# kensho-technologies/pyctcdecode

Measured on AMD Instinct MI355X. Metric: logit-frames/sec (whole node) at beam=100, V=1024, 4-gram LM, higher is better.
Workload: dtype f64

## Files before the change

### pyctcdecode_amd/csrc/backend_hip.hip

```cpp
#include <hip/hip_runtime.h>
#include <hip/hip_fp16.h>
#include <algorithm>
#include <type_traits>
#include <vector>
#include <math.h>
#include <stdio.h>
#include <stdlib.h>

#include "backend.h"
#include "beam_core.h"
#include "beam_wave.h"
#include "set_order.h"
#include "np_f32.h"
#include "set_order_small.h"
#include "np_sum.h"
#include "text_wave.h"
#include "wave_ops_hip.h"

namespace ctc {
namespace be {

static hipStream_t g_stream = nullptr;
static hipStream_t g_copy_stream = nullptr;
static hipEvent_t g_ev[3] = {nullptr, nullptr, nullptr};
// ... 1147 lines not shown
        Raw v;
        v.x = xf[e0 < V ? e0 : 0];
        v.y = xf[e0 + 1 < V ? e0 + 1 : 0];
        v.z = xf[e0 + 2 < V ? e0 + 2 : 0];
        v.w = xf[e0 + 3 < V ? e0 + 3 : 0];
        r[k] = v;
      } else {
        r[k] = x4[i4 < n4 ? i4 : 0];
      }
    }
  };
  auto widen = [&](const Raw(&raw)[NL], float4(&r)[NC]) {
    const float ninf = -INFINITY;
    if constexpr (WIDE) {
#pragma unroll
      for (int k = 0; k < NC; ++k) {
        r[k] = make_float4(raw[k].x, raw[k].y, raw[k].z, raw[k].w);
        if constexpr (!AL) {
          const int e0 = (k * 64 + lane) * 4;
          if (e0 >= V) r[k].x = ninf;
          if (e0 + 1 >= V) r[k].y = ninf;
          if (e0 + 2 >= V) r[k].z = ninf;
          if (e0 + 3 >= V) r[k].w = ninf;
        } else if (!in_row(k)) {
          r[k] = make_float4(ninf, ninf, ninf, ninf);
        }
      }
    } else {
#pragma unroll
      for (int k = 0; k < NL; ++k) {
        r[2 * k] = make_float4(pf_widen<DT>(raw[k].x & 0xFFFFu), pf_widen<DT>(raw[k].x >> 16), pf_widen<DT>(raw[k].y & 0xFFFFu),
                               pf_widen<DT>(raw[k].y >> 16));
        r[2 * k + 1] = make_float4(pf_widen<DT>(raw[k].z & 0xFFFFu), pf_widen<DT>(raw[k].z >> 16), pf_widen<DT>(raw[k].w & 0xFFFFu),
                                   pf_widen<DT>(raw[k].w >> 16));
        if (!in_row(2 * k)) {
          r[2 * k] = make_float4(ninf, ninf, ninf, ninf);
          r[2 * k + 1] = make_float4(ninf, ninf, ninf, ninf);
        }
      }
    }
  };

  float my_m = 0.f, my_rs = 0.f, my_s32 = 1.0f;
  double my_s = 1.0;
  int my_first = 0;
  uint32_t my_cnt = 0;

  int np_off0 = 0, np_len0 = 0;
  if constexpr (NP) {
    const int leaf = lane >> 3;
    if (leaf < a.np_n_leaf) {
      np_off0 = a.np_leaf[2 * leaf];
      np_len0 = a.np_leaf[2 * leaf + 1];
    }
  }
  auto np_accumulate = [&](int i) {
#ifdef CTC_NP_DIAG_NOEXCH
    if (lane < a.np_n_leaf) np_ls[lane * PF_ROWS + i] = 1.0f;
    return;
#endif
    __builtin_amdgcn_fence(__ATOMIC_SEQ_CST, "wavefront");
    __builtin_amdgcn_wave_barrier();
    const int g = lane >> 3, j = lane & 7;
    const int nl = a.np_n_leaf;
    for (int base = 0; base < nl; base += 8) {
      const int leaf = base + g;
      const bool mine = leaf < nl;
      int off = np_off0, len = np_len0;
      if (base > 0) {
        off = len = 0;
        if (mine) {
          off = a.np_leaf[2 * leaf];
          len = a.np_leaf[2 * leaf + 1];
        }
      }
      float res = 0.f;
      if (len == 128 && (off & 127) == 0) {
        const float* q = np_rb + np_pad(off) + j;
        float t0 = q[0], t1 = q[8], t2 = q[16], t3 = q[24], t4 = q[32], t5 = q[40], t6 = q[48], t7 = q[56];
        float t8 = q[64], t9 = q[72], t10 = q[80], t11 = q[88], t12 = q[96], t13 = q[104], t14 = q[112], t15 = q[120];
        float rr = t0 + t1;
        rr = rr + t2; rr = rr + t3; rr = rr + t4; rr = rr + t5; rr = rr + t6; rr = rr + t7; rr = rr + t8;
        rr = rr + t9; rr = rr + t10; rr = rr + t11; rr = rr + t12; rr = rr + t13; rr = rr + t14; rr = rr + t15;
        res = rr;
      } else if (len >= 8) {
        const int body = len - (len & 7);
        float rr = np_rb[np_pad(off + j)];
        for (int t = 8; t < body; t += 8) rr = rr + np_rb[np_pad(off + t + j)];
        res = rr;
      }
      res = res + dpp_f32<0xB1, 0xf>(0.f, res);
      res = res + dpp_f32<0x4E, 0xf>(0.f, res);
      res = res + dpp_f32<0x141, 0xf>(0.f, res);
      if ((len & 7) != 0 || len < 8) {
        const int body = len >= 8 ? len - (len & 7) : 0;
        if (len < 8) res = 0.f;
        for (int t = body; t < len; ++t) res = res + np_rb[np_pad(off + t)];
      }
      if (a.np_uniform8) {
        float t = res + dpp_f32<0x128, 0xf>(0.f, res);
        t = t + dpp_f32<0x142, 0xa>(0.f, t);
        t = t + dpp_f32<0x143, 0xc>(0.f, t);
        const float total = __int_as_float(__builtin_amdgcn_readlane(__float_as_int(t), 63));
        if (lane == i) my_s32 = total;
      } else if (mine && j == 0) {
        np_ls[leaf * PF_ROWS + i] = res;
      }
    }
    __builtin_amdgcn_fence(__ATOMIC_SEQ_CST, "wavefront");
    __builtin_amdgcn_wave_barrier();
  };

  auto phase_a = [&](int i, const Raw(&raw)[NL]) -> uint32_t {
    float4 r[NC];
    widen(raw, r);
    float mf = -INFINITY, rsf;
#pragma unroll
    for (int k = 0; k < NC; ++k) mf = max3_raw(max3_raw(mf, r[k].x, r[k].y), r[k].z, r[k].w);
    if (!AL) {
      rsf = 0.f;
#pragma unroll
      for (int k = 0; k < NC; ++k) {
        const int e0 = (k * 64 + lane) * 4;
        rsf += ((e0 < V ? r[k].x : 0.f) + (e0 + 1 < V ? r[k].y : 0.f)) + ((e0 + 2 < V ? r[k].z : 0.f) + (e0 + 3 < V ? r[k].w : 0.f));
      }
    } else if (n4 == NL * 64) {
      f32x2 rs2 = (f32x2)(0.f);
#pragma unroll
      for (int k = 0; k < NC; ++k) rs2 += (f32x2){r[k].x, r[k].y} + (f32x2){r[k].z, r[k].w};
      rsf = rs2.x + rs2.y;
    } else {
      rsf = 0.f;
#pragma unroll
      for (int k = 0; k < NC; ++k) rsf += in_row(k) ? (r[k].x + r[k].y) + (r[k].z + r[k].w) : 0.f;
    }
    const float m = wave_max_f32(mf);
    const float rs = wave_sum_f32(rsf);
    uint32_t cnt = 0xFFFFu;
    int first = 0;
    double s = 1.0;
    bool clean = isfinite(m) && rs == rs;
    if constexpr (NP) {
      float lo = INFINITY;
#pragma unroll
      for (int k = 0; k < NC; ++k) {
        if constexpr (AL) {
          if (n4 == NL * 64 || in_row(k)) lo = min3_raw(min3_raw(lo, r[k].x, r[k].y), r[k].z, r[k].w);
        } else {
          const int e0 = (k * 64 + lane) * 4;
          lo = fminf(lo, fminf(fminf(e0 < V ? r[k].x : lo, e0 + 1 < V ? r[k].y : lo), fminf(e0 + 2 < V ? r[k].z : lo, e0 + 3 < V ? r[k].w : lo)));
        }
      }
      if (clean && __ballot(!(lo - m > -87.0f)) != 0ull) clean = false;
    }
    if (clean) {
      if constexpr (NP) {
        f32x2 approx = (f32x2)(0.f);
        const f32x2 mm2 = (f32x2)(m);
#if !defined(CTC_NP_DIAG_PKEXP) && !defined(CTC_NP_CHAINWISE)
#ifndef CTC_NP_IL
#define CTC_NP_IL 2
#endif
        constexpr int IL = NC % CTC_NP_IL == 0 ? CTC_NP_IL : 1;
        f32x2 ex[NC][2];
#pragma unroll
        for (int k0 = 0; k0 < NC; k0 += IL) {
          f32x2 tin[2 * IL], tout[2 * IL];
#pragma unroll
          for (int j = 0; j < IL; ++j) {
            tin[2 * j] = (f32x2){r[k0 + j].x, r[k0 + j].y} - mm2;
            tin[2 * j + 1] = (f32x2){r[k0 + j].z, r[k0 + j].w} - mm2;
          }
          np_exp_nonpos_pk_fast_n<2 * IL>(tin, tout);
#pragma unroll
          for (int j = 0; j < IL; ++j) {
            ex[k0 + j][0] = tout[2 * j];
            ex[k0 + j][1] = tout[2 * j + 1];
          }
        }
#endif
#pragma unroll
        for (int k = 0; k < NC; ++k) {
#ifdef CTC_NP_DIAG_PKEXP
          const f32x2 e01 = exp_nonpos_f32x2m((f32x2){r[k].x, r[k].y} - mm2), e23 = exp_nonpos_f32x2m((f32x2){r[k].z, r[k].w} - mm2);
#elif defined(CTC_NP_CHAINWISE)
          const f32x2 e01 = np_exp_nonpos_pk_fast((f32x2){r[k].x, r[k].y} - mm2), e23 = np_exp_nonpos_pk_fast((f32x2){r[k].z, r[k].w} - mm2);
#else
          const f32x2 e01 = ex[k][0], e23 = ex[k][1];
#endif
          bool inside = true;
          if constexpr (AL) inside = n4 == NL * 64 || in_row(k);
          else inside = (k * 64 + lane) * 4 + 3 < V;
          if (inside) approx += e01 + e23;
#ifndef CTC_NP_DIAG_NOEXCH
          *(float4*)(np_rb + np_pad((k * 64 + lane) * 4)) = make_float4(e01.x, e01.y, e23.x, e23.y);
#endif
        }
        s = (double)wave_sum_f32(approx.x + approx.y);
      } else {
      f32x2 acc = (f32x2)(0.f);
      const f32x2 mm = (f32x2)(m);
#pragma unroll
      for (int k = 0; k < NC; ++k) {
#ifdef CTC_PF_SKIP_EXP
        acc += ((f32x2){r[k].x, r[k].y} - mm) * (f32x2)(1e-9f) + ((f32x2){r[k].z, r[k].w} - mm) * (f32x2)(1e-9f);
#else
        acc += exp_nonpos_f32x2m((f32x2){r[k].x, r[k].y} - mm);
        acc += exp_nonpos_f32x2m((f32x2){r[k].z, r[k].w} - mm);
#endif
      }
      s = wave_sum((double)(acc.x + acc.y));
#ifdef CTC_PF_SKIP_EXP
      s = 1.02 + s * 1e-30;
#endif
      }
      const float xthr = (m + __logf((float)s)) + tminf;
      const float pre = xthr - 3e-5f * (4.0f + fabsf(xthr));
      cnt = 0;
#pragma unroll
      for (int k = 0; k < NC; ++k) {
#pragma unroll
        for (int e = 0; e < 4; ++e) {
          const float x = e == 0 ? r[k].x : e == 1 ? r[k].y : e == 2 ? r[k].z : r[k].w;
          const bool c = x >= pre;
          const uint64_t mk = __ballot(c);
          if (mk) {
            const uint32_t pos = cnt + lanes_below(mk);
            if (c && pos < (uint32_t)PF_CAND) {
              ar_id[pos * PF_ROWS + i] = (uint16_t)id_of(k, e);
              ar_x[pos * PF_ROWS + i] = x;
            }
            cnt += (uint32_t)__popcll(mk);
          }
        }
      }
      if (cnt == 0) {
        first = 0x7FFFFFFF;
#pragma unroll
        for (int k = 0; k < NC; ++k) {
          if (first == 0x7FFFFFFF || (!WIDE && (k & 1))) {
            const uint64_t b0 = __ballot(r[k].x == m), b1 = __ballot(r[k].y == m), b2 = __ballot(r[k].z == m),
                           b3 = __ballot(r[k].w == m);
            const uint64_t any = b0 | b1 | b2 | b3;
            if (any) {
              const int l = __builtin_ctzll(any);
              const int e = ((b0 >> l) & 1ull) ? 0 : ((b1 >> l) & 1ull) ? 1 : ((b2 >> l) & 1ull) ? 2 : 3;
              const int cand = WIDE ? (k * 64 + l) * 4 + e : ((k >> 1) * 64 + l) * 8 + (k & 1) * 4 + e;
              if (cand < first) first = cand;
            }
          }
        }
      }
      if constexpr (NP) np_accumulate(i);
    }
    if (lane == i) {
      my_m = m;
      my_rs = rs;
      my_s = s;
      my_first = first;
      my_cnt = cnt;
    }
    return cnt;
  };

  const int64_t row_last = row_lo + nrows - 1;
  auto row_at = [&](int i) { return row_lo + i < row_last ? row_lo + i : row_last; };
  if constexpr (NC <= 4) {
    Raw ra[NL], rb[NL], rc[NL];
    load_row(row_at(0), ra);
    load_row(row_at(1), rb);
    for (int i = 0; i < nrows; i += 3) {
      load_row(row_at(i + 2), rc);
      phase_a(i, ra);
      load_row(row_at(i + 3), ra);
      if (i + 1 < nrows) phase_a(i + 1, rb);
      load_row(row_at(i + 4), rb);
      if (i + 2 < nrows) phase_a(i + 2, rc);
    }
  } else if constexpr (NC <= 8) {
    Raw ra[NL], rb[NL];
    load_row(row_at(0), ra);
    for (int i = 0; i < nrows; i += 2) {
      load_row(row_at(i + 1), rb);
      phase_a(i, ra);
      load_row(row_at(i + 2), ra);
      if (i + 1 < nrows) phase_a(i + 1, rb);
    }
  } else {
    Raw ra[NL];
    for (int i = 0; i < nrows; ++i) {
      load_row(row_at(i), ra);
      phase_a(i, ra);
    }
  }
  __syncthreads();

  const int64_t row = row_lo + lane;
  const uint32_t ms = (uint32_t)a.max_surv;
  bool slow = false;
#ifdef CTC_PF_SKIP_B
  if (lane < nrows) {
    a.surv_id[(size_t)row * ms] = 0;
    a.surv_lp[(size_t)row * ms] = -1.0 + 1e-30 * (double)(my_cnt + (uint32_t)my_first) + 1e-30 * my_s;
    a.surv_cnt[row] = 1;
    a.row_sum[row] = (double)my_rs + (double)my_m * 1e-30;
  }
#else
  if (lane < nrows) {
    const uint32_t cnt = my_cnt;
    slow = cnt > (uint32_t)PF_CAND;
    if (!slow) {
      const double s = my_s;
      const double md = (double)my_m;
      double lse = 0.0;
      float l32 = 0.f;
      if constexpr (NP) {
        float s32 = my_s32;
        if (!a.np_uniform8) {
          for (int q = 0; q + 1 < a.np_n_leaf; ++q) {
            const int dst = a.np_prog[2 * q], src = a.np_prog[2 * q + 1];
            np_ls[dst * PF_ROWS + lane] = np_ls[dst * PF_ROWS + lane] + np_ls[src * PF_ROWS + lane];
          }
          s32 = np_ls[lane];
        }
        l32 = np_log_f32(s32);
      } else {
        lse = log_ge1(s);
      }
      auto logp_of = [&](float x) { return NP ? to_logp_np32(x, false, my_m, l32) : to_logp((double)x, false, md, lse); };
      const double best = logp_of(my_m);
      uint16_t* ids = ar_id + lane;
      float* xs = ar_x + lane;
      uint32_t n = 0;
      uint32_t first = cnt > 0 ? 0xFFFFu : (uint32_t)my_first;
      for (uint32_t j = 0; j < cnt; ++j) {
        const uint16_t id = ids[j * PF_ROWS];
        const float x = xs[j * PF_ROWS];
        if (x == my_m && id < first) first = id;
        if (logp_of(x) >= a.token_min_logp) {
          uint32_t p = n;
          while (p > 0 && ids[(p - 1) * PF_ROWS] > id) {
            ids[p * PF_ROWS] = ids[(p - 1) * PF_ROWS];
            xs[p * PF_ROWS] = xs[(p - 1) * PF_ROWS];
            --p;
          }
          ids[p * PF_ROWS] = id;
          xs[p * PF_ROWS] = x;
          ++n;
        }
      }
      slow = n > SMALL_SET_MAX_KEYS || n >= ms;
      if (!slow) {
        LaneTab tab{tabs + lane};
        const SmallSet r = small_set_order(tab, n, [ids](uint32_t k) { return (uint32_t)ids[k * PF_ROWS]; },
                                           first);
        uint16_t* out_id = a.surv_id + (size_t)row * ms;
        double* out_lp = a.surv_lp + (size_t)row * ms;
        uint32_t pos = 0;
        for (uint32_t k = 0; k <= r.mask; ++k) {
          const uint16_t v = tab.get(r.base + k);
          if (v != SMALL_SET_EMPTY) {
            const uint32_t pay = v >> SMALL_SET_ID_BITS;
            out_id[pos] = (uint16_t)(v & SMALL_SET_ID_MASK);
            out_lp[pos] = pay == SMALL_SET_ARGMAX ? best : logp_of(xs[pay * PF_ROWS]);
            ++pos;
          }
        }
        a.surv_cnt[row] = pos;
        a.row_sum[row] = (double)my_rs;
      }
    }
  }
#endif
  const uint64_t sm = __ballot(slow);
  if (sm) {
    uint32_t base = 0;
    if (lane == 0) base = atomicAdd(&a.overflow[3], (uint32_t)__popcll(sm));
    base = (uint32_t)__builtin_amdgcn_readfirstlane((int)base);
    if (slow) a.slow_rows[base + lanes_below(sm)] = (uint32_t)(row - a.row_base);
  }
}

struct NpPlan {
  int V = -1, n_leaf = 0, uniform8 = 0;
  uint16_t* d_leaf = nullptr;
  uint8_t* d_prog = nullptr;
};
static int np_plan_node(int off, int n, std::vector<uint16_t>& leaf, std::vector<uint8_t>& prog) {
  if (n <= 128) {
    leaf.push_back((uint16_t)off);
    leaf.push_back((uint16_t)n);
    return (int)leaf.size() / 2 - 1;
  }
  int n2 = n / 2;
  n2 -= n2 % 8;
  const int l = np_plan_node(off, n2, leaf, prog), r = np_plan_node(off + n2, n - n2, leaf, prog);
  prog.push_back((uint8_t)l);
  prog.push_back((uint8_t)r);
  return l;
}
static int np_plan_for(int V, NpPlan** out, std::string* err) {
  static NpPlan plans[4];
  static int next = 0;
  for (NpPlan& p : plans)
    if (p.V == V) {
      *out = &p;
      return 0;
    }
  NpPlan& p = plans[next];
  next = (next + 1) % 4;
  std::vector<uint16_t> leaf;
  std::vector<uint8_t> prog;
  np_plan_node(0, V, leaf, prog);
  prog.push_back(0);
  prog.push_back(0);
  HIP_TRY(hipStreamSynchronize(g_stream));
  if (p.d_leaf) (void)hipFree(p.d_leaf);
  if (p.d_prog) (void)hipFree(p.d_prog);
  p.d_leaf = nullptr;
  p.d_prog = nullptr;
  p.V = -1;
  HIP_TRY(hipMalloc((void**)&p.d_leaf, leaf.size() * 2));
  HIP_TRY(hipMalloc((void**)&p.d_prog, prog.size()));
  HIP_TRY(hipMemcpy(p.d_leaf, leaf.data(), leaf.size() * 2, hipMemcpyHostToDevice));
  HIP_TRY(hipMemcpy(p.d_prog, prog.data(), prog.size(), hipMemcpyHostToDevice));
  p.n_leaf = (int)leaf.size() / 2;
  p.uniform8 = (p.n_leaf == 1 || p.n_leaf == 2 || p.n_leaf == 4 || p.n_leaf == 8) ? 1 : 0;
  for (size_t k = 0; k < leaf.size(); k += 2)
    if (leaf[k + 1] != 128 || (leaf[k] & 127) != 0) p.uniform8 = 0;
  p.V = V;
  *out = &p;
  return 0;
}

int launch_prune(const PruneArgs& a_in, std::string* err) {
  PruneArgs a = a_in;
  {
    const char* ex0 = getenv("CTCDEC_PRUNE_EXP");
    a.f32_np = (a.dtype == 0 && !(ex0 && (ex0[0] == 'p' || ex0[0] == 'f'))) ? 1 : 0;
    a.np_prog = nullptr;
    a.np_leaf = nullptr;
    a.np_n_leaf = 0;
    a.np_uniform8 = 0;
  }
  if (a.pass == 0) {
    g_timing_valid = false;
    HIP_TRY(hipEventRecord(g_ev[0], g_stream));
  }
  if (a.n_rows > 0) {
    uint32_t cap = set_table_cap((uint32_t)a.max_surv + 1);
    size_t lds = prune_lds_bytes((size_t)a.max_surv, cap) * PRUNE_WAVES;
    if (lds > 160 * 1024) {
      if (err) *err = "token_min_logp admits too many labels per frame for the LDS set tables";
      return -1;
    }
    dim3 grid((unsigned)((a.n_rows + PRUNE_WAVES - 1) / PRUNE_WAVES)), block(PRUNE_WAVES * 64);
    const bool vec4 = a.dtype == 0 && (a.n_labels % 4) == 0 && a.n_labels <= 1024 && a.rows_aligned16;
    static_assert(PF_MAX_LABELS - 1 <= (int)SMALL_SET_MAX_ID, "label ids must fit the small set tables");
    const bool f32_fast = a.dtype == 0 && a.n_labels <= PF_MAX_LABELS && a.rows_aligned4;
    const bool f32_al = (a.n_labels % 4) == 0 && a.rows_aligned16;
#define CTC_LAUNCH_PRUNE(KERN)                                                                                 \
  do {                                                                                                         \
    HIP_TRY(hipFuncSetAttribute((const void*)KERN, hipFuncAttributeMaxDynamicSharedMemorySize, (int)lds));      \
    hipLaunchKernelGGL(KERN, grid, block, lds, g_stream, a, cap);                                              \
  } while (0)
    const char* ex = getenv("CTCDEC_PRUNE_EXP");
    const char* pk = getenv("CTCDEC_PRUNE_KERNEL");
    const bool rows_ok = a.pass == 0 && a.slow_rows && a.n_rows < (1ll << 32) && !(ex && ex[0] == 'f') && !(pk && pk[0] == 'r') &&
                         !(a.dense_hint && a.dtype == 0 && a.f32_np);
    const bool rows64 = f32_fast && rows_ok;
    const bool rows64h = (a.dtype == 2 || a.dtype == 3) && (a.n_labels % 8) == 0 && a.n_labels <= 1024 && a.rows_aligned16 && rows_ok;
    const dim3 fgrid((unsigned)((a.n_rows + PF_ROWS - 1) / PF_ROWS)), fblock(64);
    const unsigned rest = (unsigned)std::min<int64_t>((a.n_rows + PRUNE_WAVES - 1) / PRUNE_WAVES, 2048);
    if (rows64) {
      const int nc = ((a.n_labels + 3) / 4 + 63) / 64;
      size_t flds = PF_LDS;
      if (a.f32_np) {
        NpPlan* plan = nullptr;
        if (np_plan_for(a.n_labels, &plan, err)) return -1;
        a.np_leaf = plan->d_leaf;
        a.np_prog = plan->d_prog;
        a.np_n_leaf = plan->n_leaf;
        a.np_uniform8 = plan->uniform8;
        flds += pf_np_extra_lds(nc <= 8 ? nc : (nc <= 12 ? 12 : 16), plan->uniform8 ? 0 : plan->n_leaf);
      }
#define CTC_LAUNCH_FAST_K(KERN)                                                                                           \
  do {                                                                                                                    \
    HIP_TRY(hipFuncSetAttribute((const void*)KERN, hipFuncAttributeMaxDynamicSharedMemorySize, (int)flds));               \
    hipLaunchKernelGGL(KERN, fgrid, fblock, flds, g_stream, a);                                                           \
  } while (0)
#define CTC_LAUNCH_FAST(NCV, ALV)                                                                                         \
  do {                                                                                                                    \
    if (a.f32_np) CTC_LAUNCH_FAST_K((frame_prune_fast<NCV, 0, ALV, true>));                                               \
    else CTC_LAUNCH_FAST_K((frame_prune_fast<NCV, 0, ALV, false>));                                                       \
    if (ALV && NCV <= 4) {                                                                                                \
      HIP_TRY(hipFuncSetAttribute((const void*)frame_prune_f32x4_listed<(NCV <= 4 ? NCV : 4)>,                            \
                                  hipFuncAttributeMaxDynamicSharedMemorySize, (int)lds));                                 \
      hipLaunchKernelGGL((frame_prune_f32x4_listed<(NCV <= 4 ? NCV : 4)>), dim3(rest), block, lds, g_stream, a, cap);     \
    } else {                                                                                                              \
      HIP_TRY(hipFuncSetAttribute((const void*)frame_prune_listed<float>, hipFuncAttributeMaxDynamicSharedMemorySize,     \
                                  (int)lds));                                                                             \
      hipLaunchKernelGGL((frame_prune_listed<float>), dim3(rest), block, lds, g_stream, a, cap);                          \
    }                                                                                                                     \
  } while (0)
#define CTC_LAUNCH_FAST_NC(NCV)            \
  do {                                     \
    if (f32_al) CTC_LAUNCH_FAST(NCV, true); \
    else CTC_LAUNCH_FAST(NCV, false);      \
  } while (0)
      switch (nc) {
        case 1: CTC_LAUNCH_FAST_NC(1); break;
        case 2: CTC_LAUNCH_FAST_NC(2); break;
        case 3: CTC_LAUNCH_FAST_NC(3); break;
        case 4: CTC_LAUNCH_FAST_NC(4); break;
        case 5: CTC_LAUNCH_FAST_NC(5); break;
        case 6: CTC_LAUNCH_FAST_NC(6); break;
        case 7: CTC_LAUNCH_FAST_NC(7); break;
        case 8: CTC_LAUNCH_FAST_NC(8); break;
        case 9: case 10: case 11: case 12: CTC_LAUNCH_FAST_NC(12); break;
        default: CTC_LAUNCH_FAST_NC(16); break;
      }
#undef CTC_LAUNCH_FAST_NC
#undef CTC_LAUNCH_FAST
#undef CTC_LAUNCH_FAST_K
    } else if (rows64h) {
      const int nl = (a.n_labels / 8 + 63) / 64;
#define CTC_LAUNCH_FAST16(NCV, DTV, T)                                                                                    \
  do {                                                                                                                    \
    hipLaunchKernelGGL((frame_prune_fast<NCV, DTV>), fgrid, fblock, PF_LDS, g_stream, a);                                 \
    HIP_TRY(hipFuncSetAttribute((const void*)frame_prune_listed<T>, hipFuncAttributeMaxDynamicSharedMemorySize, (int)lds)); \
    hipLaunchKernelGGL((frame_prune_listed<T>), dim3(rest), block, lds, g_stream, a, cap);                                 \
  } while (0)
      if (a.dtype == 2) {
        if (nl <= 1) CTC_LAUNCH_FAST16(2, 2, half_bits);
        else CTC_LAUNCH_FAST16(4, 2, half_bits);
      } else {
        if (nl <= 1) CTC_LAUNCH_FAST16(2, 3, bf16_bits);
        else CTC_LAUNCH_FAST16(4, 3, bf16_bits);
      }
#undef CTC_LAUNCH_FAST16
    } else if (vec4) {
      const int nc = (a.n_labels / 4 + 63) / 64;
      if (!(ex && ex[0] == 'f')) {
        if (nc <= 1) CTC_LAUNCH_PRUNE((frame_prune_f32x4<1, true>));
        else if (nc == 2) CTC_LAUNCH_PRUNE((frame_prune_f32x4<2, true>));
        else if (nc == 3) CTC_LAUNCH_PRUNE((frame_prune_f32x4<3, true>));
        else CTC_LAUNCH_PRUNE((frame_prune_f32x4<4, true>));
      } else {
        if (nc <= 1) CTC_LAUNCH_PRUNE((frame_prune_f32x4<1, false>));
        else if (nc == 2) CTC_LAUNCH_PRUNE((frame_prune_f32x4<2, false>));
        else if (nc == 3) CTC_LAUNCH_PRUNE((frame_prune_f32x4<3, false>));
        else CTC_LAUNCH_PRUNE((frame_prune_f32x4<4, false>));
      }
    } else if (a.dtype == 0) {
      CTC_LAUNCH_PRUNE(frame_prune<float>);
    } else if (a.dtype == 1) {
      CTC_LAUNCH_PRUNE(frame_prune<double>);
    } else if (a.dtype == 2) {
      CTC_LAUNCH_PRUNE(frame_prune<half_bits>);
    } else {
      CTC_LAUNCH_PRUNE(frame_prune<bf16_bits>);
    }
#undef CTC_LAUNCH_PRUNE
    HIP_TRY(hipGetLastError());
  }
  if (a.n_utts > 0) {
    if (a.pass == 0) hipLaunchKernelGGL(utt_sniff, dim3((unsigned)a.n_utts), dim3(64), 0, g_stream, a);
    else hipLaunchKernelGGL(utt_recount, dim3((unsigned)a.n_utts), dim3(64), 0, g_stream, a);
    HIP_TRY(hipGetLastError());
  }
  HIP_TRY(hipEventRecord(g_ev[1], g_stream));
  return 0;
}

int launch_sniff_exact(const PruneArgs& a, std::string* err) {
  if (a.n_utts > 0) {
    hipLaunchKernelGGL(utt_sniff_exact, dim3((unsigned)a.n_utts), dim3(256), 0, g_stream, a);
    HIP_TRY(hipGetLastError());
  }
  return 0;
}

int launch_group(const BeamArgs& a, const LdsShape& shape, size_t lds, int kind, hipStream_t stream, std::string* err);
int launch_wave(const BeamArgs& a, hipStream_t stream, std::string* err);

struct TextGpuCtx {
  int lane;
  __device__ __forceinline__ void wsync() {
    __builtin_amdgcn_fence(__ATOMIC_SEQ_CST, "wavefront");
    __builtin_amdgcn_wave_barrier();
  }
  __device__ __forceinline__ uint64_t ballot(bool p) { return __ballot(p); }
  __device__ __forceinline__ int clz64(uint64_t x) { return __clzll((long long)x); }
  __device__ __forceinline__ uint32_t wave_excl_sum_u32(uint32_t v) {
    uint32_t incl = v;
#pragma unroll
    for (int off = 1; off < 64; off <<= 1) {
      const uint32_t o = (uint32_t)__shfl_up((int)incl, off, 64);
      if (lane >= off) incl += o;
    }
    return incl - v;
  }
  __device__ __forceinline__ uint32_t wave_sum_u32(uint32_t v) {
    int x = (int)v;
    x += __builtin_amdgcn_update_dpp(0, x, 0x111, 0xf, 0xf, false);
    x += __builtin_amdgcn_update_dpp(0, x, 0x112, 0xf, 0xf, false);
    x += __builtin_amdgcn_update_dpp(0, x, 0x114, 0xf, 0xf, false);
    x += __builtin_amdgcn_update_dpp(0, x, 0x118, 0xf, 0xf, false);
    x += __builtin_amdgcn_update_dpp(0, x, 0x142, 0xa, 0xf, false);
    x += __builtin_amdgcn_update_dpp(0, x, 0x143, 0xc, 0xf, false);
    return (uint32_t)__builtin_amdgcn_readlane(x, 63);
  }
};

__global__ __launch_bounds__(64) void assemble_texts(BeamArgs a) {
  __shared__ __attribute__((aligned(16))) char smem[TEXT_LDS_BYTES];
  const int u = blockIdx.x;
  const int lane = threadIdx.x;
  if (a.n_out[u] == 0) return;
  OutBeam& ob = a.out[(size_t)u * a.out_stride];
  uint8_t* scratch = a.text_scratch + a.text_soff[u];
  const uint32_t cap = (uint32_t)(a.text_soff[u + 1] - a.text_soff[u]);
  TextLds L;
  text_lds_carve(L, (CTC_LDS char*)smem);
  TextGpuCtx ctx{lane};
  const uint32_t pos = wave_text_backwards(ctx, L, a.emit_nodes + a.emit_off[u], a.tables, ob.pad[1], scratch, cap,
                                           (uint32_t)(a.emit_off[u + 1] - a.emit_off[u]));
  uint32_t len = cap - pos;
  unsigned long long base = 0;
  if (lane == 0) {
    base = atomicAdd(a.tok_pool_head + 1, (unsigned long long)len);
    if (base + len > a.text_pool_cap) {
      a.status[u] |= ST_TOK_OVERFLOW;
      base = 0;
      len = 0;
    }
    ob.tok_off = (uint32_t)base;
    ob.tok_cnt = len;
    ob.pad[0] = (uint32_t)(base >> 32);
  }
  __builtin_amdgcn_fence(__ATOMIC_SEQ_CST, "workgroup");
  __builtin_amdgcn_wave_barrier();
  len = (uint32_t)__builtin_amdgcn_readfirstlane((int)len);
  const uint32_t blo = (uint32_t)__builtin_amdgcn_readfirstlane((int)(uint32_t)base);
  const uint32_t bhi = (uint32_t)__builtin_amdgcn_readfirstlane((int)(uint32_t)(base >> 32));
  base = ((unsigned long long)bhi << 32) | blo;
  for (uint32_t k = (uint32_t)lane; k < len; k += 64u) a.text_pool[base + k] = scratch[pos + k];
}

constexpr float WEIGH_C0 = 4.0f;
constexpr float WEIGH_GAIN = 4.0f;
constexpr int PLACE_MAX = 8192;
struct WeighArgs {
  const int64_t* utt_row0;
  const uint32_t* surv_cnt;
  int32_t n_utts;
  float* total;
  float* per_frame;
  const int32_t* given_order;
  int32_t* order;
  float* block_weight;
  int32_t simds;
  float gain;
  int32_t snake;
};
__global__ __launch_bounds__(64) void utt_weigh(WeighArgs a) {
  const int u = blockIdx.x;
  const int lane = threadIdx.x;
// ... 349 lines not shown
```

### pyctcdecode_amd/csrc/set_order_small.h

```cpp
#pragma once
#include <stdint.h>

#include "common.h"

namespace ctc {

constexpr uint32_t SMALL_SET_MAX_KEYS = 15;
constexpr uint32_t SMALL_SET_SLOTS = 48;
constexpr uint16_t SMALL_SET_EMPTY = 0xFFFFu;
constexpr uint32_t SMALL_SET_ARGMAX = 15;
constexpr uint32_t SMALL_SET_ID_BITS = 12;
constexpr uint32_t SMALL_SET_ID_MASK = (1u << SMALL_SET_ID_BITS) - 1u;
constexpr uint32_t SMALL_SET_MAX_ID = SMALL_SET_ID_MASK - 1u;
static_assert(SMALL_SET_MAX_KEYS <= SMALL_SET_ARGMAX, "an index must not read as the argmax marker");

struct SmallSet {
  uint32_t base, mask, used;
};

template <class Tab>
CTC_HD void small_set_clear(Tab& tab, uint32_t base, uint32_t size) {
  for (uint32_t k = 0; k < size; ++k) tab.put(base + k, SMALL_SET_EMPTY);
}

template <class Tab>
CTC_HD void small_set_insert_clean(Tab& tab, const SmallSet& s, uint16_t entry) {
  const uint32_t key = entry & SMALL_SET_ID_MASK, mask = s.mask;
  uint32_t perturb = key, i = key & mask;
  for (;;) {
    if (tab.get(s.base + i) == SMALL_SET_EMPTY) {
      tab.put(s.base + i, entry);
      return;
    }
    if (i + 9 <= mask) {
      for (uint32_t j = 1; j <= 9; ++j)
        if (tab.get(s.base + i + j) == SMALL_SET_EMPTY) {
          tab.put(s.base + i + j, entry);
          return;
        }
    }
    perturb >>= 5;
    i = (i * 5 + 1 + perturb) & mask;
  }
}

template <class Tab>
CTC_HD bool small_set_add(Tab& tab, const SmallSet& s, uint16_t entry) {
  const uint32_t key = entry & SMALL_SET_ID_MASK, mask = s.mask;
  uint32_t perturb = key, i = key & mask;
  for (;;) {
    uint32_t probes = (i + 9 <= mask) ? 9u : 0u;
    uint32_t e = i;
    for (;;) {
      const uint16_t cur = tab.get(s.base + e);
      if (cur == SMALL_SET_EMPTY) {
        tab.put(s.base + e, entry);
        return true;
      }
      if ((cur & SMALL_SET_ID_MASK) == key) return false;
      ++e;
      if (probes == 0) break;
      --probes;
    }
    perturb >>= 5;
    i = (i * 5 + 1 + perturb) & mask;
  }
}

template <class Tab>
CTC_HD void small_set_rebuild(Tab& tab, const SmallSet& from, SmallSet& to, uint32_t to_base, uint32_t to_size) {
  small_set_clear(tab, to_base, to_size);
  to.base = to_base;
  to.mask = to_size - 1;
  to.used = from.used;
  for (uint32_t k = 0; k <= from.mask; ++k) {
    const uint16_t v = tab.get(from.base + k);
    if (v != SMALL_SET_EMPTY) small_set_insert_clean(tab, to, v);
  }
}

template <class Tab, class IdAt>
CTC_HD SmallSet small_set_order(Tab& tab, uint32_t n, IdAt id_at, uint32_t argmax) {
  SmallSet s{0, 7, 0};
  small_set_clear(tab, 0, 8);
  for (uint32_t k = 0; k < n; ++k) {
    small_set_add(tab, s, (uint16_t)(id_at(k) | (k << SMALL_SET_ID_BITS)));
    s.used += 1;
    if (s.used * 5 >= s.mask * 3) {
      SmallSet grown;
      small_set_rebuild(tab, s, grown, 16, 32);
      s = grown;
    }
  }
  if (s.used >= 5 && s.used <= 7) {
    SmallSet copy;
    small_set_rebuild(tab, s, copy, 0, 16);
    s = copy;
  } else if (s.used == 4) {
    SmallSet grown;
    small_set_rebuild(tab, s, grown, 16, 16);
    s = grown;
  }
  if (small_set_add(tab, s, (uint16_t)(argmax | (SMALL_SET_ARGMAX << SMALL_SET_ID_BITS)))) s.used += 1;
  return s;
}

}
```

Before: 186.2 million.

## Use occupancy bitmask small-set and register-resident candidates in prefilter phase B

Replaces the table-scanning small hash set with a version that tracks slot occupancy in a 32-bit mask, so inserts, rebuilds and output iteration use ctz on the mask instead of reading LDS slots. Candidates and sorted ids are loaded into registers, insertion sort skips shifting when ids arrive ascending, and a precomputed argmax-membership flag avoids a probe. For the NP path the kept value is stored pre-normalized and widened with a clip, which avoids recomputing logp. It also adds an optional debug store path under a skip macro. The risks are more register pressure from the unrolled arrays, and the assumption that duplicate-free inserts are valid (insert_clean replaces add).

```diff
diff --git a/pyctcdecode_amd/csrc/backend_hip.hip b/pyctcdecode_amd/csrc/backend_hip.hip
--- a/pyctcdecode_amd/csrc/backend_hip.hip
+++ b/pyctcdecode_amd/csrc/backend_hip.hip
@@ -1473,6 +1473,12 @@
   if (lane < nrows) {
     a.surv_id[(size_t)row * ms] = 0;
     a.surv_lp[(size_t)row * ms] = -1.0 + 1e-30 * (double)(my_cnt + (uint32_t)my_first) + 1e-30 * my_s;
+#ifdef CTC_PF_SKIP_B_STORES
+    for (uint32_t k = 1; k <= (uint32_t)CTC_PF_SKIP_B_STORES && k < ms; ++k) {
+      a.surv_id[(size_t)row * ms + k] = (uint16_t)k;
+      a.surv_lp[(size_t)row * ms + k] = -1.0 - (double)k;
+    }
+#endif
     a.surv_cnt[row] = 1;
     a.row_sum[row] = (double)my_rs + (double)my_m * 1e-30;
   }
@@ -1498,43 +1504,93 @@
       } else {
         lse = log_ge1(s);
       }
+      const double clip_lo = -34.538776394910684;
+      auto widen_clip = [&](float y32) {
+        const double y = (double)y32;
+        return y < clip_lo ? clip_lo : (y > 0.0 ? 0.0 : y);
+      };
       auto logp_of = [&](float x) { return NP ? to_logp_np32(x, false, my_m, l32) : to_logp((double)x, false, md, lse); };
       const double best = logp_of(my_m);
       uint16_t* ids = ar_id + lane;
       float* xs = ar_x + lane;
-      uint32_t n = 0;
+      uint32_t cid[PF_CAND];
+      float cx[PF_CAND];
+#pragma unroll
+      for (int j = 0; j < PF_CAND; ++j) {
+        cid[j] = ids[j * PF_ROWS];
+        cx[j] = xs[j * PF_ROWS];
+      }
+      uint32_t n = 0, top = 0;
       uint32_t first = cnt > 0 ? 0xFFFFu : (uint32_t)my_first;
-      for (uint32_t j = 0; j < cnt; ++j) {
-        const uint16_t id = ids[j * PF_ROWS];
-        const float x = xs[j * PF_ROWS];
-        if (x == my_m && id < first) first = id;
-        if (logp_of(x) >= a.token_min_logp) {
-          uint32_t p = n;
-          while (p > 0 && ids[(p - 1) * PF_ROWS] > id) {
-            ids[p * PF_ROWS] = ids[(p - 1) * PF_ROWS];
-            xs[p * PF_ROWS] = xs[(p - 1) * PF_ROWS];
-            --p;
+#pragma unroll
+      for (int j = 0; j < PF_CAND; ++j) {
+        if (__ballot((uint32_t)j < cnt) == 0ull) break;
+        if ((uint32_t)j < cnt) {
+          const uint32_t id = cid[j];
+          const float x = cx[j];
+          if (x == my_m && id < first) first = id;
+          float keep = x;
+          double lp;
+          if constexpr (NP) {
+            const float t = x - my_m;
+            keep = t - l32;
+            lp = widen_clip(keep);
+          } else {
+            lp = logp_of(x);
           }
-          ids[p * PF_ROWS] = id;
-          xs[p * PF_ROWS] = x;
-          ++n;
+          if (lp >= a.token_min_logp) {
+            uint32_t p = n;
+            if (n > 0 && id < top) {
+              while (p > 0 && ids[(p - 1) * PF_ROWS] > id) {
+                ids[p * PF_ROWS] = ids[(p - 1) * PF_ROWS];
+                xs[p * PF_ROWS] = xs[(p - 1) * PF_ROWS];
+                --p;
+              }
+            } else {
+              top = id;
+            }
+            ids[p * PF_ROWS] = (uint16_t)id;
+            xs[p * PF_ROWS] = keep;
+            ++n;
+          }
         }
       }
       slow = n > SMALL_SET_MAX_KEYS || n >= ms;
       if (!slow) {
+        uint32_t sid[SMALL_SET_MAX_KEYS];
+#pragma unroll
+        for (uint32_t k = 0; k < SMALL_SET_MAX_KEYS; ++k) sid[k] = ids[k * PF_ROWS];
+        bool member = false;
+#pragma unroll
+        for (uint32_t k = 0; k < SMALL_SET_MAX_KEYS; ++k) member = member || (k < n && sid[k] == first);
         LaneTab tab{tabs + lane};
-        const SmallSet r = small_set_order(tab, n, [ids](uint32_t k) { return (uint32_t)ids[k * PF_ROWS]; },
-                                           first);
+        const SmallSetBits r = small_set_order_bits(tab, n, [&sid](uint32_t k) { return sid[k]; }, first, member ? 1 : 0);
         uint16_t* out_id = a.surv_id + (size_t)row * ms;
         double* out_lp = a.surv_lp + (size_t)row * ms;
-        uint32_t pos = 0;
-        for (uint32_t k = 0; k <= r.mask; ++k) {
-          const uint16_t v = tab.get(r.base + k);
-          if (v != SMALL_SET_EMPTY) {
-            const uint32_t pay = v >> SMALL_SET_ID_BITS;
-            out_id[pos] = (uint16_t)(v & SMALL_SET_ID_MASK);
-            out_lp[pos] = pay == SMALL_SET_ARGMAX ? best : logp_of(xs[pay * PF_ROWS]);
-            ++pos;
+        const uint32_t pos = r.used;
+        constexpr int OUT_MAX = (int)SMALL_SET_MAX_KEYS + 1;
+        uint32_t ov[OUT_MAX];
+        float okept[OUT_MAX];
+        uint32_t left = r.occ;
+#pragma unroll
+        for (int p = 0; p < OUT_MAX; ++p) {
+          if (__ballot((uint32_t)p < pos) == 0ull) break;
+          ov[p] = tab.get(r.base + (left ? small_set_ctz(left) : 0u));
+          left &= left - 1;
+        }
+#pragma unroll
+        for (int p = 0; p < OUT_MAX; ++p) {
+          if (__ballot((uint32_t)p < pos) == 0ull) break;
+          const uint32_t pay = ov[p] >> SMALL_SET_ID_BITS;
+          okept[p] = xs[(pay >= SMALL_SET_ARGMAX ? 0u : pay) * PF_ROWS];
+        }
+#pragma unroll
+        for (int p = 0; p < OUT_MAX; ++p) {
+          if (__ballot((uint32_t)p < pos) == 0ull) break;
+          if ((uint32_t)p < pos) {
+            const uint32_t pay = ov[p] >> SMALL_SET_ID_BITS;
+            out_id[p] = (uint16_t)(ov[p] & SMALL_SET_ID_MASK);
+            out_lp[p] = pay == SMALL_SET_ARGMAX ? best : NP ? widen_clip(okept[p]) : logp_of(okept[p]);
           }
         }
         a.surv_cnt[row] = pos;
diff --git a/pyctcdecode_amd/csrc/set_order_small.h b/pyctcdecode_amd/csrc/set_order_small.h
--- a/pyctcdecode_amd/csrc/set_order_small.h
+++ b/pyctcdecode_amd/csrc/set_order_small.h
@@ -105,4 +105,115 @@
   return s;
 }
 
-}
+struct SmallSetBits {
+  uint32_t base, mask, used, occ;
+};
+
+CTC_HD uint32_t small_set_ctz(uint32_t v) {
+#if defined(__HIP_DEVICE_COMPILE__)
+  return (uint32_t)__ffs((int)v) - 1u;
+#else
+  return (uint32_t)__builtin_ctz(v);
+#endif
+}
+
+template <class Tab>
+CTC_HD void small_set_insert_clean_bits(Tab& tab, SmallSetBits& s, uint16_t entry) {
+  const uint32_t key = entry & SMALL_SET_ID_MASK, mask = s.mask;
+  uint32_t perturb = key, i = key & mask;
+  for (;;) {
+    const uint32_t window = (i + 9 <= mask) ? 0x3FFu : 1u;
+    const uint32_t free = ~(s.occ >> i) & window;
+    if (free) {
+      const uint32_t e = i + small_set_ctz(free);
+      tab.put(s.base + e, entry);
+      s.occ |= 1u << e;
+      return;
+    }
+    perturb >>= 5;
+    i = (i * 5 + 1 + perturb) & mask;
+  }
+}
+
+template <class Tab>
+CTC_HD bool small_set_add_bits(Tab& tab, SmallSetBits& s, uint16_t entry) {
+  const uint32_t key = entry & SMALL_SET_ID_MASK, mask = s.mask;
+  uint32_t perturb = key, i = key & mask;
+  for (;;) {
+    uint32_t probes = (i + 9 <= mask) ? 9u : 0u;
+    uint32_t e = i;
+    for (;;) {
+      if (((s.occ >> e) & 1u) == 0) {
+        tab.put(s.base + e, entry);
+        s.occ |= 1u << e;
+        return true;
+      }
+      if ((tab.get(s.base + e) & SMALL_SET_ID_MASK) == key) return false;
+      ++e;
+      if (probes == 0) break;
+      --probes;
+    }
+    perturb >>= 5;
+    i = (i * 5 + 1 + perturb) & mask;
+  }
+}
+
+#if defined(__clang__)
+#define CTC_SMALL_SET_UNROLL _Pragma("unroll")
+#else
+#define CTC_SMALL_SET_UNROLL
+#endif
+constexpr uint32_t SMALL_SET_MOVED_MAX = 7;
+
+template <class Tab>
+CTC_HD void small_set_rebuild_bits(Tab& tab, const SmallSetBits& from, SmallSetBits& to, uint32_t to_base, uint32_t to_size) {
+  to.base = to_base;
+  to.mask = to_size - 1;
+  to.used = from.used;
+  to.occ = 0;
+  uint16_t moved[SMALL_SET_MOVED_MAX];
+  uint32_t left = from.occ;
+  CTC_SMALL_SET_UNROLL
+  for (uint32_t i = 0; i < SMALL_SET_MOVED_MAX; ++i) {
+    moved[i] = tab.get(from.base + (left ? small_set_ctz(left) : 0u));
+    left &= left - 1;
+  }
+  CTC_SMALL_SET_UNROLL
+  for (uint32_t i = 0; i < SMALL_SET_MOVED_MAX; ++i)
+    if (i < from.used) small_set_insert_clean_bits(tab, to, moved[i]);
+}
+
+template <class Tab, class IdAt>
+CTC_HD SmallSetBits small_set_order_bits(Tab& tab, uint32_t n, IdAt id_at, uint32_t argmax, int member = -1) {
+  SmallSetBits s{0, 7, 0, 0};
+  CTC_SMALL_SET_UNROLL
+  for (uint32_t k = 0; k < SMALL_SET_MAX_KEYS; ++k) {
+    if (k >= n) break;
+    small_set_insert_clean_bits(tab, s, (uint16_t)(id_at(k) | (k << SMALL_SET_ID_BITS)));
+    s.used += 1;
+    if (k == 4) {
+      SmallSetBits grown;
+      small_set_rebuild_bits(tab, s, grown, 16, 32);
+      s = grown;
+    }
+  }
+  if (s.used >= 5 && s.used <= 7) {
+    SmallSetBits copy;
+    small_set_rebuild_bits(tab, s, copy, 0, 16);
+    s = copy;
+  } else if (s.used == 4) {
+    SmallSetBits grown;
+    small_set_rebuild_bits(tab, s, grown, 16, 16);
+    s = grown;
+  }
+  const uint16_t entry = (uint16_t)(argmax | (SMALL_SET_ARGMAX << SMALL_SET_ID_BITS));
+  if (member < 0) {
+    if (small_set_add_bits(tab, s, entry)) s.used += 1;
+  } else if (member == 0) {
+    small_set_insert_clean_bits(tab, s, entry);
+    s.used += 1;
+  }
+  return s;
+}
+
+}
```

Result: slower. 182.1 million (-2.2%).
